# rapidsai/distributed-join

Hardware: NVIDIA H100
Metric: joined rows/sec (build+probe rows through distributed_inner_join) at 400Mx400M int64 (higher is better)
Workload: dtype int64

## Files before the change

### distributed-join_b200/csrc/join.cu

```cuda
#include <algorithm>
#include <cstdlib>
#include <type_traits>

#include "dj_device.cuh"
#include "dj_internal.h"

namespace dj {

namespace {

template <int THREADS, int SLOTS, int BUILD_CHUNK, int TARGET_ROWS, int PROBE_STAGES, int OUT_ROWS>
struct JoinCfg {
  static constexpr int kThreads     = THREADS;
  static constexpr int kConsumers   = THREADS - 32;
  static constexpr int kConsWarps   = kConsumers / 32;
  static constexpr int kSlots       = SLOTS;
  static constexpr int kBuildChunk  = BUILD_CHUNK;
  static constexpr int kTargetRows  = TARGET_ROWS;
  static constexpr int kProbeChunk  = kConsumers;
  static constexpr int kProbeStages = PROBE_STAGES;
  static constexpr int kOutRows     = OUT_ROWS;
};
using CfgA = JoinCfg<1024, 8192, 1792, 1536, 2, 576>;
using CfgB = JoinCfg<512, 4096, 1024, 768, 2, 256>;

constexpr int kOutTiles    = 3;
constexpr int kDescBuckets = 128;

struct JoinDev {
  const Row* build;
  const int64_t *bbeg, *bend;
  const Row* probe;
  const int64_t *pbeg, *pend;
  int nbuckets;
  int64_t* out[4];
  int64_t out_capacity;
  unsigned long long* out_count;
  uint32_t* probe_bits;
  uint8_t* out_sides;
  uint32_t* build_bits;
};

constexpr int kInner = 0, kSemi = DJ_JOIN_LEFT_SEMI, kAnti = DJ_JOIN_LEFT_ANTI;
constexpr int kLeftOuter = DJ_JOIN_LEFT_OUTER, kFullOuter = DJ_JOIN_FULL_OUTER, kMark = kJoinFullOuterMark;
constexpr uint8_t kSideProbe = DJ_SIDE_LEFT, kSideBuild = DJ_SIDE_RIGHT;

__host__ __device__ constexpr bool is_outer(int kind)
{
  return kind == kLeftOuter || kind == kFullOuter || kind == kMark;
}
__host__ __device__ constexpr bool marks_build(int kind) { return kind == kFullOuter || kind == kMark; }

template <class C>
struct __align__(128) JoinSmem {
  uint32_t slots[2][C::kSlots];
  Row brow[2][C::kBuildChunk];
  Row prow[C::kProbeStages][C::kProbeChunk];
  int64_t sout[kOutTiles][4][C::kOutRows];
  int64_t dbb[kDescBuckets], dbe[kDescBuckets];
  int64_t dpb[kDescBuckets], dpe[kDescBuckets];
  unsigned long long full_build[2], empty_build[2];
  unsigned long long full_probe[C::kProbeStages], empty_probe[C::kProbeStages];
  unsigned long long sbase[kOutTiles];
  int scnt[kOutTiles];
};

template <class C>
struct __align__(128) OuterJoinSmem : JoinSmem<C> {
  uint8_t ssides[kOutTiles][C::kOutRows];
  uint32_t bmatch[2][C::kBuildChunk / 32];
};

template <class C, int KIND>
using JoinSmemOf = std::conditional_t<is_outer(KIND), OuterJoinSmem<C>, JoinSmem<C>>;

template <int N>
__device__ __forceinline__ void consumer_sync()
{
  asm volatile("bar.sync 1, %0;" ::"n"(N) : "memory");
}

template <int KIND, class S>
__device__ __forceinline__ int next_valid_bucket(const S& s, int lb, int nd)
{
  if constexpr (KIND == kAnti || KIND == kLeftOuter || KIND == kMark) {
    while (lb < nd && s.dpe[lb] == s.dpb[lb]) lb++;
  } else if constexpr (KIND == kFullOuter) {
    while (lb < nd && s.dbe[lb] == s.dbb[lb] && s.dpe[lb] == s.dpb[lb]) lb++;
  } else {
    while (lb < nd && (s.dbe[lb] == s.dbb[lb] || s.dpe[lb] == s.dpb[lb])) lb++;
  }
  return lb;
}

__device__ __forceinline__ uint32_t slot_tag(uint32_t h) { return 0x100000u | (h >> 12); }

template <class C>
__device__ __forceinline__ void emit_outer_row(OuterJoinSmem<C>& s, const JoinDev& d, int cur, int lane, bool emit,
                                               int64_t bk, int64_t bp, int64_t pk, int64_t pv, uint8_t sides)
{
  const unsigned m = __ballot_sync(0xffffffffu, emit);
  if (m == 0) return;
  const int leader = __ffs(m) - 1;
  int obase        = 0;
  if (lane == leader) {
    obase = atomicAdd(&s.scnt[cur], __popc(m));
    if (obase >= C::kOutRows) atomicSub(&s.scnt[cur], __popc(m));
  }
  obase            = __shfl_sync(0xffffffffu, obase, leader);
  const int pos    = obase + __popc(m & lanemask_lt());
  const bool spill = emit && pos >= C::kOutRows;
  if (emit && !spill) {
    s.sout[cur][0][pos] = bk;
    s.sout[cur][1][pos] = bp;
    s.sout[cur][2][pos] = pk;
    s.sout[cur][3][pos] = pv;
    s.ssides[cur][pos]  = sides;
  }
  const unsigned ms = __ballot_sync(0xffffffffu, spill);
  if (ms) {
    const int sl         = __ffs(ms) - 1;
    unsigned long long g = 0;
    if (lane == sl) g = atomicAdd(d.out_count, (unsigned long long)__popc(ms));
    g = __shfl_sync(0xffffffffu, g, sl);
    if (spill) {
      const int64_t gi = (int64_t)g + __popc(ms & lanemask_lt());
      if (gi < d.out_capacity) {
        d.out[0][gi]     = bk;
        d.out[1][gi]     = bp;
        d.out[2][gi]     = pk;
        d.out[3][gi]     = pv;
        d.out_sides[gi]  = sides;
      }
    }
  }
}

template <class C, int KIND>
__global__ void __launch_bounds__(C::kThreads, 1) bucket_join_kernel(JoinDev d)
{
  using Smem = JoinSmemOf<C, KIND>;
  constexpr int kConsumers = C::kConsumers;
  constexpr bool kOuter    = is_outer(KIND);
  constexpr bool kEmptyJob = KIND == kAnti || kOuter;
  constexpr int kCols      = (KIND == kSemi || KIND == kAnti) ? 2 : 4;
  extern __shared__ __align__(128) unsigned char smem_raw[];
  Smem& s        = *reinterpret_cast<Smem*>(smem_raw);
  const int tid  = threadIdx.x;
  const int lane = tid & 31;
  const int warp = tid >> 5;
  const bool is_producer = warp == C::kConsWarps;

  if (tid == 0) {
    for (int i = 0; i < 2; i++) {
      mbar_init(&s.full_build[i], 1);
      mbar_init(&s.empty_build[i], C::kConsWarps);
    }
    for (int i = 0; i < C::kProbeStages; i++) {
      mbar_init(&s.full_probe[i], 1);
      mbar_init(&s.empty_probe[i], C::kConsWarps);
    }
    for (int i = 0; i < kOutTiles; i++) s.scnt[i] = 0;
    asm volatile("fence.mbarrier_init.release.cluster;" ::: "memory");
  }
  for (int i = tid; i < 2 * C::kSlots; i += C::kThreads) (&s.slots[0][0])[i] = 0;
  if constexpr (marks_build(KIND))
    for (int i = tid; i < 2 * (C::kBuildChunk / 32); i += C::kThreads) (&s.bmatch[0][0])[i] = 0;
  __syncthreads();

  const int lo = (int)((int64_t)d.nbuckets * blockIdx.x / gridDim.x);
  const int hi = (int)((int64_t)d.nbuckets * (blockIdx.x + 1) / gridDim.x);

  uint32_t q = 0;
  uint32_t u = 0;
  int cur = 0, pend_tile = 0, pend_n = 0;
  unsigned long long pend_base_reg = 0;

  for (int base = lo; base < hi; base += kDescBuckets) {
    const int nd = min(kDescBuckets, hi - base);
    __syncthreads();
    for (int i = tid; i < nd; i += C::kThreads) {
      s.dbb[i] = d.bbeg[base + i];
      s.dbe[i] = d.bend[base + i];
      s.dpb[i] = d.pbeg[base + i];
      s.dpe[i] = d.pend[base + i];
    }
    __syncthreads();

    if (is_producer) {
      if (lane == 0) {
        for (int lb = next_valid_bucket<KIND>(s, 0, nd); lb < nd; lb = next_valid_bucket<KIND>(s, lb + 1, nd)) {
          const int64_t b0 = s.dbb[lb], b1 = s.dbe[lb], p0 = s.dpb[lb], p1 = s.dpe[lb];
          for (int64_t c0 = b0; c0 < b1 || (kEmptyJob && c0 == b0); c0 += C::kBuildChunk) {
            {
              const int bs = u & 1;
              const int n  = (int)min((int64_t)C::kBuildChunk, b1 - c0);
              mbar_wait(&s.empty_build[bs], ((u >> 1) & 1) ^ 1);
              mbar_expect_tx(&s.full_build[bs], (uint32_t)n * 16u);
              if (!kEmptyJob || n > 0) tma_load(s.brow[bs], d.build + c0, (uint32_t)n * 16u, &s.full_build[bs]);
              u++;
            }
            for (int64_t r0 = p0; r0 < p1; r0 += C::kProbeChunk) {
              const int st = q % C::kProbeStages;
              const int n  = (int)min((int64_t)C::kProbeChunk, p1 - r0);
              mbar_wait(&s.empty_probe[st], ((q / C::kProbeStages) & 1) ^ 1);
              mbar_expect_tx(&s.full_probe[st], (uint32_t)n * 16u);
              tma_load(s.prow[st], d.probe + r0, (uint32_t)n * 16u, &s.full_probe[st]);
              q++;
            }
          }
        }
      }
      __syncwarp();
    } else {
      for (int lb = next_valid_bucket<KIND>(s, 0, nd); lb < nd; lb = next_valid_bucket<KIND>(s, lb + 1, nd)) {
        const int64_t b0 = s.dbb[lb], b1 = s.dbe[lb], p0 = s.dpb[lb], p1 = s.dpe[lb];
        const bool multi = KIND != kInner && b1 - b0 > C::kBuildChunk;
        for (int64_t c0 = b0; c0 < b1 || (kEmptyJob && c0 == b0); c0 += C::kBuildChunk) {
          const bool last = c0 + C::kBuildChunk >= b1;
          const int bs = u & 1;
          const int nb = (int)min((int64_t)C::kBuildChunk, b1 - c0);
          uint32_t* slots     = s.slots[bs];
          const Row* brow     = s.brow[bs];
          mbar_wait(&s.full_build[bs], (u >> 1) & 1);
          for (int r = tid; r < nb; r += kConsumers) {
            const uint32_t h = slot_hash_i64(brow[r].key);
            const uint32_t e = (slot_tag(h) << 11) | (uint32_t)r;
            uint32_t slot    = h & (C::kSlots - 1);
            while (atomicCAS(&slots[slot], 0u, e) != 0u) slot = (slot + 1) & (C::kSlots - 1);
          }
          {
            uint4* other = reinterpret_cast<uint4*>(s.slots[bs ^ 1]);
            for (int i = tid; i < C::kSlots / 4; i += kConsumers) other[i] = make_uint4(0, 0, 0, 0);
            if constexpr (KIND == kFullOuter)
              for (int i = tid; i < C::kBuildChunk / 32; i += kConsumers) s.bmatch[bs ^ 1][i] = 0;
          }
          consumer_sync<kConsumers>();

          for (int64_t r0 = p0; r0 < p1; r0 += C::kProbeChunk) {
            const int st = q % C::kProbeStages;
            const int np = (int)min((int64_t)C::kProbeChunk, p1 - r0);
            mbar_wait(&s.full_probe[st], (q / C::kProbeStages) & 1);
            bool alive = tid < np;
            int64_t k = 0, v = 0;
            if (alive) {
              const int4 pr = *reinterpret_cast<const int4*>(&s.prow[st][tid]);
              k = (int64_t)(((uint64_t)(uint32_t)pr.y << 32) | (uint32_t)pr.x);
              v = (int64_t)(((uint64_t)(uint32_t)pr.w << 32) | (uint32_t)pr.z);
            }
            const unsigned landed =
              __reduce_and_sync(0xffffffffu, (uint32_t)((uint64_t)k ^ ((uint64_t)k >> 32) ^ (uint64_t)v ^
                                                        ((uint64_t)v >> 32)) | 1u);
            if (lane == 0 && landed) mbar_arrive(&s.empty_probe[st]);
            q++;

            const uint32_t h    = slot_hash_i64(k);
            const uint32_t want = slot_tag(h);
            uint32_t slot       = h & (C::kSlots - 1);
            if constexpr (kOuter) {
              const bool valid = alive;
              bool matched     = false;
              while (true) {
                bool found = false;
                int idx    = 0;
                if (alive) {
                  while (true) {
                    const uint32_t e = slots[slot];
                    if (e == 0u) {
                      alive = false;
                      break;
                    }
                    if ((e >> 11) == want) {
                      idx = (int)(e & 0x7ffu);
                      if (brow[idx].key == k) {
                        found = true;
                        break;
                      }
                    }
                    slot = (slot + 1) & (C::kSlots - 1);
                  }
                }
                if (!__any_sync(0xffffffffu, found)) break;
                int64_t bpay = 0;
                if (found) {
                  matched = true;
                  bpay    = brow[idx].pay;
                  if constexpr (marks_build(KIND)) {
                    uint32_t* w      = &s.bmatch[bs][idx >> 5];
                    const uint32_t b = 1u << (idx & 31);
                    if (!(*w & b)) atomicOr(w, b);
                  }
                }
                emit_outer_row<C>(s, d, cur, lane, found, k, bpay, k, v, kSideBuild | kSideProbe);
                if (found) slot = (slot + 1) & (C::kSlots - 1);
              }
              const int64_t prow_at = r0 + tid;
              uint32_t* word        = d.probe_bits + (prow_at >> 5);
              const uint32_t bit    = 1u << (prow_at & 31);
              if (multi && matched && !last) atomicOr(word, bit);
              const bool lone = valid && !matched && last && (!multi || !(__ldcg(word) & bit));
              emit_outer_row<C>(s, d, cur, lane, lone, 0, 0, k, v, kSideProbe);
              continue;
            }
            if constexpr (KIND == kSemi || KIND == kAnti) {
              bool found = false;
              if (alive) {
                while (true) {
                  const uint32_t e = slots[slot];
                  if (e == 0u) break;
                  if ((e >> 11) == want && brow[e & 0x7ffu].key == k) {
                    found = true;
                    break;
                  }
                  slot = (slot + 1) & (C::kSlots - 1);
                }
              }
              const int64_t prow_at = r0 + tid;
              uint32_t* word        = d.probe_bits + (prow_at >> 5);
              const uint32_t bit    = 1u << (prow_at & 31);
              bool emit;
              if constexpr (KIND == kSemi) {
                emit = found && (!multi || !(atomicOr(word, bit) & bit));
              } else {
                if (multi && found && !last) atomicOr(word, bit);
                emit = alive && !found && last && (!multi || !(__ldcg(word) & bit));
              }
              const unsigned m = __ballot_sync(0xffffffffu, emit);
              if (m) {
                const int leader = __ffs(m) - 1;
                int obase        = 0;
                if (lane == leader) {
                  obase = atomicAdd(&s.scnt[cur], __popc(m));
                  if (obase >= C::kOutRows) atomicSub(&s.scnt[cur], __popc(m));
                }
                obase            = __shfl_sync(0xffffffffu, obase, leader);
                const int pos    = obase + __popc(m & lanemask_lt());
                const bool spill = emit && pos >= C::kOutRows;
                if (emit && !spill) {
                  s.sout[cur][0][pos] = k;
                  s.sout[cur][1][pos] = v;
                }
                const unsigned ms = __ballot_sync(0xffffffffu, spill);
                if (ms) {
                  const int sl = __ffs(ms) - 1;
                  unsigned long long g = 0;
                  if (lane == sl) g = atomicAdd(d.out_count, (unsigned long long)__popc(ms));
                  g = __shfl_sync(0xffffffffu, g, sl);
                  if (spill) {
                    const int64_t gi = (int64_t)g + __popc(ms & lanemask_lt());
                    if (gi < d.out_capacity) {
                      d.out[0][gi] = k;
                      d.out[1][gi] = v;
                    }
                  }
                }
              }
              continue;
            }
            while (true) {
              bool found = false;
              int idx    = 0;
              if (alive) {
                while (true) {
                  const uint32_t e = slots[slot];
                  if (e == 0u) {
                    alive = false;
                    break;
                  }
                  if ((e >> 11) == want) {
                    idx = (int)(e & 0x7ffu);
                    if (brow[idx].key == k) {
                      found = true;
                      break;
                    }
                  }
                  slot = (slot + 1) & (C::kSlots - 1);
                }
              }
              const unsigned m = __ballot_sync(0xffffffffu, found);
              if (m == 0) break;
              const int leader = __ffs(m) - 1;
              int obase        = 0;
              if (lane == leader) {
                obase = atomicAdd(&s.scnt[cur], __popc(m));
                if (obase >= C::kOutRows) atomicSub(&s.scnt[cur], __popc(m));
              }
              obase         = __shfl_sync(0xffffffffu, obase, leader);
              const int pos = obase + __popc(m & lanemask_lt());
              const bool spill = found && pos >= C::kOutRows;
              if (found && !spill) {
                s.sout[cur][0][pos] = k;
                s.sout[cur][1][pos] = brow[idx].pay;
                s.sout[cur][2][pos] = k;
                s.sout[cur][3][pos] = v;
              }
              const unsigned ms = __ballot_sync(0xffffffffu, spill);
              if (ms) {
                const int sl = __ffs(ms) - 1;
                unsigned long long g = 0;
                if (lane == sl) g = atomicAdd(d.out_count, (unsigned long long)__popc(ms));
                g = __shfl_sync(0xffffffffu, g, sl);
                if (spill) {
                  const int64_t gi = (int64_t)g + __popc(ms & lanemask_lt());
                  if (gi < d.out_capacity) {
                    d.out[0][gi] = k;
                    d.out[1][gi] = brow[idx].pay;
                    d.out[2][gi] = k;
                    d.out[3][gi] = v;
                  }
                }
              }
              if (found) slot = (slot + 1) & (C::kSlots - 1);
            }
          }

          if (tid == 0 && pend_n) s.sbase[pend_tile] = pend_base_reg;
          consumer_sync<kConsumers>();
          if constexpr (KIND == kFullOuter) {
            for (int r0 = tid - lane; r0 < nb; r0 += kConsumers) {
              const int r     = r0 + lane;
              const bool lone = r < nb && !((s.bmatch[bs][r >> 5] >> (r & 31)) & 1u);
              int64_t bk = 0, bp = 0;
              if (lone) {
                bk = brow[r].key;
                bp = brow[r].pay;
              }
              emit_outer_row<C>(s, d, cur, lane, lone, bk, bp, 0, 0, kSideBuild);
            }
            consumer_sync<kConsumers>();
          }
          if constexpr (KIND == kMark) {
            if (tid < C::kBuildChunk / 32) {
              const uint32_t w = s.bmatch[bs][tid];
              if (w) {
                s.bmatch[bs][tid] = 0;
                const int64_t at  = c0 + 32 * tid;
                uint32_t* g       = d.build_bits + (at >> 5);
                const int sh      = (int)(at & 31);
                atomicOr(g, w << sh);
                if (sh && (w >> (32 - sh))) atomicOr(g + 1, w >> (32 - sh));
              }
            }
          }
          if (lane == 0) mbar_arrive(&s.empty_build[bs]);
          if (pend_n) {
            const int64_t gb = (int64_t)s.sbase[pend_tile];
#pragma unroll
            for (int c = 0; c < kCols; c++)
              for (int i = tid; i < pend_n; i += kConsumers)
                if (gb + i < d.out_capacity) d.out[c][gb + i] = s.sout[pend_tile][c][i];
            if constexpr (kOuter)
              for (int i = tid; i < pend_n; i += kConsumers)
                if (gb + i < d.out_capacity) d.out_sides[gb + i] = s.ssides[pend_tile][i];
            if (tid == 0) s.scnt[pend_tile] = 0;
            pend_n = 0;
          }
          int n_out = s.scnt[cur];
          if (n_out > 0) {
            if (n_out > C::kOutRows) n_out = C::kOutRows;
            if (tid == 0) pend_base_reg = atomicAdd(d.out_count, (unsigned long long)n_out);
            pend_n    = n_out;
            pend_tile = cur;
            cur       = cur + 1 == kOutTiles ? 0 : cur + 1;
          }
          u++;
        }
      }
    }
  }

  if (!is_producer) {
    if (tid == 0 && pend_n) s.sbase[pend_tile] = pend_base_reg;
    consumer_sync<kConsumers>();
    if (pend_n) {
      const int64_t gb = (int64_t)s.sbase[pend_tile];
#pragma unroll
      for (int c = 0; c < kCols; c++)
        for (int i = tid; i < pend_n; i += kConsumers)
          if (gb + i < d.out_capacity) d.out[c][gb + i] = s.sout[pend_tile][c][i];
      if constexpr (kOuter)
        for (int i = tid; i < pend_n; i += kConsumers)
          if (gb + i < d.out_capacity) d.out_sides[gb + i] = s.ssides[pend_tile][i];
    }
  }
}

int join_shape()
{
  static int shape = -1;
  if (shape < 0) {
    const char* e = getenv("DJ_JOIN_SHAPE");
    shape         = (e && (e[0] == 'B' || e[0] == 'b')) ? 1 : 0;
  }
  return shape;
}

template <class C, int KIND>
int launch_join(const JoinDev& d, int ctas_per_sm, cudaStream_t stream)
{
  const size_t smem = sizeof(JoinSmemOf<C, KIND>);
  auto kern         = bucket_join_kernel<C, KIND>;
  DJ_CUDA_TRY(cudaFuncSetAttribute(kern, cudaFuncAttributeMaxDynamicSharedMemorySize, (int)smem));
  int grid = sm_count() * ctas_per_sm;
  if (grid > d.nbuckets) grid = d.nbuckets;
  {
    ProfScope prof(DJ_PROF_JOIN, stream);
    kern<<<grid, C::kThreads, smem, stream>>>(d);
  }
  DJ_LAUNCH_CHECK();
  return DJ_OK;
}

template <class C>
int launch_join_kind(const JoinDev& d, int kind, int ctas_per_sm, cudaStream_t stream)
{
  return kind == kSemi        ? launch_join<C, kSemi>(d, ctas_per_sm, stream)
         : kind == kAnti      ? launch_join<C, kAnti>(d, ctas_per_sm, stream)
         : kind == kLeftOuter ? launch_join<C, kLeftOuter>(d, ctas_per_sm, stream)
         : kind == kFullOuter ? launch_join<C, kFullOuter>(d, ctas_per_sm, stream)
         : kind == kMark      ? launch_join<C, kMark>(d, ctas_per_sm, stream)
                              : launch_join<C, kInner>(d, ctas_per_sm, stream);
}

constexpr int kAppendChunk = 4096;

__global__ void __launch_bounds__(256) append_rows_kernel(const Row* rows, const int64_t* sb, const int64_t* se,
                                                          int64_t* out_key, int64_t* out_pay, int64_t* null_key,
                                                          int64_t* null_pay, uint8_t* out_sides, uint8_t sides,
                                                          int64_t out_capacity, unsigned long long* out_count)
{
  __shared__ unsigned long long base;
  const int64_t b = sb[blockIdx.y], e = se[blockIdx.y];
  for (int64_t c0 = b + (int64_t)blockIdx.x * kAppendChunk; c0 < e; c0 += (int64_t)gridDim.x * kAppendChunk) {
    const int n = (int)min((int64_t)kAppendChunk, e - c0);
    __syncthreads();
    if (threadIdx.x == 0) base = atomicAdd(out_count, (unsigned long long)n);
    __syncthreads();
    for (int i = threadIdx.x; i < n; i += blockDim.x) {
      const int64_t g = (int64_t)base + i;
      if (g < out_capacity) {
        const Row r = rows[c0 + i];
        out_key[g]  = r.key;
        out_pay[g]  = r.pay;
        if (out_sides) {
          null_key[g]  = 0;
          null_pay[g]  = 0;
          out_sides[g] = sides;
        }
      }
    }
  }
}

constexpr int kEmitThreads = 256, kEmitPerThread = 4, kEmitTile = kEmitThreads * kEmitPerThread;

__global__ void __launch_bounds__(kEmitThreads) emit_unmatched_build_kernel(
  const Row* rows, const int64_t* bbeg, const int64_t* bend, int nbuckets, const uint32_t* bits, int64_t* null_key,
  int64_t* null_pay, int64_t* out_key, int64_t* out_pay, uint8_t* out_sides, int64_t out_capacity,
  unsigned long long* out_count)
{
  constexpr int kRuns = kEmitTile / 32;
  __shared__ unsigned long long run_base[kRuns];
  __shared__ int run_cnt[kRuns];
  const int lane = threadIdx.x & 31, warp = threadIdx.x >> 5;
  for (int b = blockIdx.x; b < nbuckets; b += gridDim.x) {
    const int64_t b0 = bbeg[b], b1 = bend[b];
    for (int64_t t0 = b0; t0 < b1; t0 += kEmitTile) {
      int4 row[kEmitPerThread];
      unsigned lone[kEmitPerThread];
#pragma unroll
      for (int j = 0; j < kEmitPerThread; j++) {
        const int64_t r = t0 + j * kEmitThreads + threadIdx.x;
        bool mine       = false;
        row[j]          = make_int4(0, 0, 0, 0);
        if (r < b1 && !((bits[r >> 5] >> (r & 31)) & 1u)) {
          mine   = true;
          row[j] = __ldg(reinterpret_cast<const int4*>(rows + r));
        }
        lone[j] = __ballot_sync(0xffffffffu, mine);
        if (lane == 0) run_cnt[j * (kEmitThreads / 32) + warp] = __popc(lone[j]);
      }
      __syncthreads();
      if (warp == 0) {
        int c[kRuns / 32], sum = 0;
#pragma unroll
        for (int i = 0; i < kRuns / 32; i++) {
          c[i] = run_cnt[lane * (kRuns / 32) + i];
          sum += c[i];
        }
        int incl = sum;
#pragma unroll
        for (int o = 1; o < 32; o <<= 1) {
          const int v = __shfl_up_sync(0xffffffffu, incl, o);
          if (lane >= o) incl += v;
        }
        const int total      = __shfl_sync(0xffffffffu, incl, 31);
        unsigned long long g = 0;
        if (lane == 0 && total) g = atomicAdd(out_count, (unsigned long long)total);
        g = __shfl_sync(0xffffffffu, g, 0) + (unsigned long long)(incl - sum);
#pragma unroll
        for (int i = 0; i < kRuns / 32; i++) {
          run_base[lane * (kRuns / 32) + i] = g;
          g += c[i];
        }
      }
      __syncthreads();
#pragma unroll
      for (int j = 0; j < kEmitPerThread; j++) {
        if (!((lone[j] >> lane) & 1u)) continue;
        const int64_t g = (int64_t)run_base[j * (kEmitThreads / 32) + warp] + __popc(lone[j] & lanemask_lt());
        if (g < out_capacity) {
          null_key[g]  = 0;
          null_pay[g]  = 0;
          out_key[g]   = (int64_t)(((uint64_t)(uint32_t)row[j].y << 32) | (uint32_t)row[j].x);
          out_pay[g]   = (int64_t)(((uint64_t)(uint32_t)row[j].w << 32) | (uint32_t)row[j].z);
          out_sides[g] = kSideBuild;
        }
      }
    }
  }
}

}

RadixPlan make_radix_plan(int64_t nbuild)
{
  const int target = join_shape() == 1 ? CfgB::kTargetRows : CfgA::kTargetRows;
  RadixPlan p{0, 0, 1};
  int bits = 0;
  while (bits < 20 && (nbuild >> bits) > target) bits++;
  if (bits <= 10) {
    p.bits1 = bits;
    p.bits2 = 0;
  } else {
    p.bits1 = bits / 2;
    p.bits2 = bits - p.bits1;
  }
  p.nbuckets = 1 << bits;
  return p;
}

int run_bucket_join(const JoinBuffers& jb, bool swap_output_sides, cudaStream_t stream)
{
  JoinDev d{};
  d.build    = jb.build;
  d.bbeg     = jb.d_build_begin;
  d.bend     = jb.d_build_end;
  d.probe    = jb.probe;
  d.pbeg     = jb.d_probe_begin;
  d.pend     = jb.d_probe_end;
  d.nbuckets = jb.nbuckets;
  for (int c = 0; c < 4; c++) d.out[c] = jb.out[swap_output_sides ? (c + 2) % 4 : c];
  d.out_capacity = jb.out_capacity;
  d.out_count    = (unsigned long long*)jb.d_out_count;
  d.probe_bits   = jb.d_probe_bits;
  d.out_sides    = jb.out_sides;
  d.build_bits   = jb.d_build_bits;
  return join_shape() == 1 ? launch_join_kind<CfgB>(d, jb.kind, 2, stream)
                           : launch_join_kind<CfgA>(d, jb.kind, 1, stream);
}

int append_segment_rows(const Row* rows, const int64_t* d_seg_begin, const int64_t* d_seg_end, int nseg,
                        int64_t max_seg_rows, int64_t* out_key, int64_t* out_pay, int64_t out_capacity,
                        int64_t* d_out_count, cudaStream_t stream, int64_t* null_key, int64_t* null_pay,
                        uint8_t* out_sides, uint8_t sides)
{
  if (nseg <= 0 || max_seg_rows <= 0) return DJ_OK;
  const int64_t chunks = (max_seg_rows + kAppendChunk - 1) / kAppendChunk;
  const dim3 grid((unsigned)(chunks < 64 ? chunks : 64), (unsigned)nseg);
  {
    ProfScope prof(DJ_PROF_OTHER, stream);
    append_rows_kernel<<<grid, 256, 0, stream>>>(rows, d_seg_begin, d_seg_end, out_key, out_pay, null_key, null_pay,
                                                 out_sides, sides, out_capacity, (unsigned long long*)d_out_count);
  }
  DJ_LAUNCH_CHECK();
  return DJ_OK;
}

int emit_unmatched_build(const Row* rows, const int64_t* d_begin, const int64_t* d_end, int nbuckets,
                         const uint32_t* d_build_bits, int64_t* const out[4], uint8_t* out_sides,
                         int64_t out_capacity, int64_t* d_out_count, cudaStream_t stream)
{
  if (nbuckets <= 0) return DJ_OK;
  const int grid = std::min(nbuckets, sm_count() * 8);
  {
    ProfScope prof(DJ_PROF_OTHER, stream);
    emit_unmatched_build_kernel<<<grid, kEmitThreads, 0, stream>>>(rows, d_begin, d_end, nbuckets, d_build_bits, out[0],
                                                                   out[1], out[2], out[3], out_sides, out_capacity,
                                                                   (unsigned long long*)d_out_count);
  }
  DJ_LAUNCH_CHECK();
  return DJ_OK;
}

const void* join_module_kernel() { return (const void*)bucket_join_kernel<CfgA, kInner>; }

}
```

Measured before the change: 25.06 billion.

## Split join CTA into independent producer/consumer groups processing interleaved buckets

Reorganizes the bucket join kernel so that a 1024-thread CTA becomes two independent 512-thread groups. Each group has its own hash slots, build buffer, probe stages, mbarriers and output tile, and takes every other valid bucket. Double-buffered build chunks and the three-tile output ring are replaced by one buffer per group, with the output tile flushed at the start of the next chunk. The aim is to cut CTA-wide synchronisation and let two pipelines overlap their latency, at the cost of losing build double-buffering within a group and adding more serialising group barriers.

```diff
diff --git a/distributed-join_b200/csrc/join.cu b/distributed-join_b200/csrc/join.cu
--- a/distributed-join_b200/csrc/join.cu
+++ b/distributed-join_b200/csrc/join.cu
@@ -9,22 +9,23 @@
 
 namespace {
 
-template <int THREADS, int SLOTS, int BUILD_CHUNK, int TARGET_ROWS, int PROBE_STAGES, int OUT_ROWS>
+template <int GROUPS, int SLOTS, int BUILD_CHUNK, int TARGET_ROWS, int PROBE_STAGES, int OUT_ROWS>
 struct JoinCfg {
-  static constexpr int kThreads     = THREADS;
-  static constexpr int kConsumers   = THREADS - 32;
-  static constexpr int kConsWarps   = kConsumers / 32;
-  static constexpr int kSlots       = SLOTS;
-  static constexpr int kBuildChunk  = BUILD_CHUNK;
-  static constexpr int kTargetRows  = TARGET_ROWS;
-  static constexpr int kProbeChunk  = kConsumers;
-  static constexpr int kProbeStages = PROBE_STAGES;
-  static constexpr int kOutRows     = OUT_ROWS;
+  static constexpr int kGroups       = GROUPS;
+  static constexpr int kGroupThreads = 512;
+  static constexpr int kThreads      = GROUPS * kGroupThreads;
+  static constexpr int kConsumers    = kGroupThreads - 32;
+  static constexpr int kConsWarps    = kConsumers / 32;
+  static constexpr int kSlots        = SLOTS;
+  static constexpr int kBuildChunk   = BUILD_CHUNK;
+  static constexpr int kTargetRows   = TARGET_ROWS;
+  static constexpr int kProbeChunk   = kConsumers;
+  static constexpr int kProbeStages  = PROBE_STAGES;
+  static constexpr int kOutRows      = OUT_ROWS;
 };
-using CfgA = JoinCfg<1024, 8192, 1792, 1536, 2, 576>;
-using CfgB = JoinCfg<512, 4096, 1024, 768, 2, 256>;
-
-constexpr int kOutTiles    = 3;
+using CfgA = JoinCfg<2, 8192, 1792, 1536, 2, 1024>;
+using CfgB = JoinCfg<1, 4096, 1024, 768, 2, 512>;
+
 constexpr int kDescBuckets = 128;
 
 struct JoinDev {
@@ -52,32 +53,40 @@
 __host__ __device__ constexpr bool marks_build(int kind) { return kind == kFullOuter || kind == kMark; }
 
 template <class C>
+struct __align__(128) JoinGroup {
+  uint32_t slots[C::kSlots];
+  Row brow[C::kBuildChunk];
+  Row prow[C::kProbeStages][C::kProbeChunk];
+  int64_t sout[4][C::kOutRows];
+  unsigned long long full_build, empty_build;
+  unsigned long long full_probe[C::kProbeStages], empty_probe[C::kProbeStages];
+  unsigned long long sbase;
+  int scnt;
+};
+
+template <class C>
+struct __align__(128) OuterJoinGroup : JoinGroup<C> {
+  uint8_t ssides[C::kOutRows];
+  uint32_t bmatch[C::kBuildChunk / 32];
+};
+
+template <class C, int KIND>
+using JoinGroupOf = std::conditional_t<is_outer(KIND), OuterJoinGroup<C>, JoinGroup<C>>;
+
+template <class C, int KIND>
 struct __align__(128) JoinSmem {
-  uint32_t slots[2][C::kSlots];
-  Row brow[2][C::kBuildChunk];
-  Row prow[C::kProbeStages][C::kProbeChunk];
-  int64_t sout[kOutTiles][4][C::kOutRows];
+  JoinGroupOf<C, KIND> grp[C::kGroups];
   int64_t dbb[kDescBuckets], dbe[kDescBuckets];
   int64_t dpb[kDescBuckets], dpe[kDescBuckets];
-  unsigned long long full_build[2], empty_build[2];
-  unsigned long long full_probe[C::kProbeStages], empty_probe[C::kProbeStages];
-  unsigned long long sbase[kOutTiles];
-  int scnt[kOutTiles];
 };
 
-template <class C>
-struct __align__(128) OuterJoinSmem : JoinSmem<C> {
-  uint8_t ssides[kOutTiles][C::kOutRows];
-  uint32_t bmatch[2][C::kBuildChunk / 32];
-};
-
-template <class C, int KIND>
-using JoinSmemOf = std::conditional_t<is_outer(KIND), OuterJoinSmem<C>, JoinSmem<C>>;
-
 template <int N>
-__device__ __forceinline__ void consumer_sync()
-{
-  asm volatile("bar.sync 1, %0;" ::"n"(N) : "memory");
+__device__ __forceinline__ void group_sync(int g)
+{
+  if (g == 0)
+    asm volatile("bar.sync 1, %0;" ::"n"(N) : "memory");
+  else
+    asm volatile("bar.sync 2, %0;" ::"n"(N) : "memory");
 }
 
 template <int KIND, class S>
@@ -93,10 +102,18 @@
   return lb;
 }
 
+template <class C, int KIND, class S>
+__device__ __forceinline__ int next_group_bucket(const S& s, int lb, int nd, uint32_t& ord, int g)
+{
+  for (lb = next_valid_bucket<KIND>(s, lb, nd); lb < nd; lb = next_valid_bucket<KIND>(s, lb + 1, nd))
+    if (ord++ % C::kGroups == (uint32_t)g) break;
+  return lb;
+}
+
 __device__ __forceinline__ uint32_t slot_tag(uint32_t h) { return 0x100000u | (h >> 12); }
 
 template <class C>
-__device__ __forceinline__ void emit_outer_row(OuterJoinSmem<C>& s, const JoinDev& d, int cur, int lane, bool emit,
+__device__ __forceinline__ void emit_outer_row(OuterJoinGroup<C>& s, const JoinDev& d, int lane, bool emit,
                                                int64_t bk, int64_t bp, int64_t pk, int64_t pv, uint8_t sides)
 {
   const unsigned m = __ballot_sync(0xffffffffu, emit);
@@ -104,18 +121,18 @@
   const int leader = __ffs(m) - 1;
   int obase        = 0;
   if (lane == leader) {
-    obase = atomicAdd(&s.scnt[cur], __popc(m));
-    if (obase >= C::kOutRows) atomicSub(&s.scnt[cur], __popc(m));
+    obase = atomicAdd(&s.scnt, __popc(m));
+    if (obase >= C::kOutRows) atomicSub(&s.scnt, __popc(m));
   }
   obase            = __shfl_sync(0xffffffffu, obase, leader);
   const int pos    = obase + __popc(m & lanemask_lt());
   const bool spill = emit && pos >= C::kOutRows;
   if (emit && !spill) {
-    s.sout[cur][0][pos] = bk;
-    s.sout[cur][1][pos] = bp;
-    s.sout[cur][2][pos] = pk;
-    s.sout[cur][3][pos] = pv;
-    s.ssides[cur][pos]  = sides;
+    s.sout[0][pos] = bk;
+    s.sout[1][pos] = bp;
+    s.sout[2][pos] = pk;
+    s.sout[3][pos] = pv;
+    s.ssides[pos]  = sides;
   }
   const unsigned ms = __ballot_sync(0xffffffffu, spill);
   if (ms) {
@@ -137,44 +154,57 @@
 }
 
 template <class C, int KIND>
+__device__ __forceinline__ void copy_out_tile(const JoinGroupOf<C, KIND>& s, const JoinDev& d, int n, int ltid)
+{
+  constexpr int kCols = (KIND == kSemi || KIND == kAnti) ? 2 : 4;
+  const int64_t gb    = (int64_t)s.sbase;
+#pragma unroll
+  for (int c = 0; c < kCols; c++)
+    for (int i = ltid; i < n; i += C::kConsumers)
+      if (gb + i < d.out_capacity) d.out[c][gb + i] = s.sout[c][i];
+  if constexpr (is_outer(KIND))
+    for (int i = ltid; i < n; i += C::kConsumers)
+      if (gb + i < d.out_capacity) d.out_sides[gb + i] = s.ssides[i];
+}
+
+template <class C, int KIND>
 __global__ void __launch_bounds__(C::kThreads, 1) bucket_join_kernel(JoinDev d)
 {
-  using Smem = JoinSmemOf<C, KIND>;
+  using Smem = JoinSmem<C, KIND>;
   constexpr int kConsumers = C::kConsumers;
   constexpr bool kOuter    = is_outer(KIND);
   constexpr bool kEmptyJob = KIND == kAnti || kOuter;
-  constexpr int kCols      = (KIND == kSemi || KIND == kAnti) ? 2 : 4;
   extern __shared__ __align__(128) unsigned char smem_raw[];
   Smem& s        = *reinterpret_cast<Smem*>(smem_raw);
   const int tid  = threadIdx.x;
   const int lane = tid & 31;
-  const int warp = tid >> 5;
-  const bool is_producer = warp == C::kConsWarps;
-
-  if (tid == 0) {
-    for (int i = 0; i < 2; i++) {
-      mbar_init(&s.full_build[i], 1);
-      mbar_init(&s.empty_build[i], C::kConsWarps);
+  const int g    = tid / C::kGroupThreads;
+  const int ltid = tid % C::kGroupThreads;
+  const bool is_producer = ltid >= kConsumers;
+  auto& sg = s.grp[g];
+
+  if (ltid == 0) {
+    mbar_init(&sg.full_build, 1);
+    mbar_init(&sg.empty_build, C::kConsWarps);
+    for (int i = 0; i < C::kProbeStages; i++) {
+      mbar_init(&sg.full_probe[i], 1);
+      mbar_init(&sg.empty_probe[i], C::kConsWarps);
     }
-    for (int i = 0; i < C::kProbeStages; i++) {
-      mbar_init(&s.full_probe[i], 1);
-      mbar_init(&s.empty_probe[i], C::kConsWarps);
-    }
-    for (int i = 0; i < kOutTiles; i++) s.scnt[i] = 0;
+    sg.scnt = 0;
     asm volatile("fence.mbarrier_init.release.cluster;" ::: "memory");
   }
-  for (int i = tid; i < 2 * C::kSlots; i += C::kThreads) (&s.slots[0][0])[i] = 0;
+  for (int i = ltid; i < C::kSlots; i += C::kGroupThreads) sg.slots[i] = 0;
   if constexpr (marks_build(KIND))
-    for (int i = tid; i < 2 * (C::kBuildChunk / 32); i += C::kThreads) (&s.bmatch[0][0])[i] = 0;
+    for (int i = ltid; i < C::kBuildChunk / 32; i += C::kGroupThreads) sg.bmatch[i] = 0;
   __syncthreads();
 
   const int lo = (int)((int64_t)d.nbuckets * blockIdx.x / gridDim.x);
   const int hi = (int)((int64_t)d.nbuckets * (blockIdx.x + 1) / gridDim.x);
 
-  uint32_t q = 0;
-  uint32_t u = 0;
-  int cur = 0, pend_tile = 0, pend_n = 0;
-  unsigned long long pend_base_reg = 0;
+  uint32_t ord = 0;
+  uint32_t q   = 0;
+  uint32_t u   = 0;
+  int pend_n = 0;
 
   for (int base = lo; base < hi; base += kDescBuckets) {
     const int nd = min(kDescBuckets, hi - base);
@@ -189,23 +219,23 @@
 
     if (is_producer) {
       if (lane == 0) {
-        for (int lb = next_valid_bucket<KIND>(s, 0, nd); lb < nd; lb = next_valid_bucket<KIND>(s, lb + 1, nd)) {
+        for (int lb = next_group_bucket<C, KIND>(s, 0, nd, ord, g); lb < nd;
+             lb     = next_group_bucket<C, KIND>(s, lb + 1, nd, ord, g)) {
           const int64_t b0 = s.dbb[lb], b1 = s.dbe[lb], p0 = s.dpb[lb], p1 = s.dpe[lb];
           for (int64_t c0 = b0; c0 < b1 || (kEmptyJob && c0 == b0); c0 += C::kBuildChunk) {
             {
-              const int bs = u & 1;
-              const int n  = (int)min((int64_t)C::kBuildChunk, b1 - c0);
-              mbar_wait(&s.empty_build[bs], ((u >> 1) & 1) ^ 1);
-              mbar_expect_tx(&s.full_build[bs], (uint32_t)n * 16u);
-              if (!kEmptyJob || n > 0) tma_load(s.brow[bs], d.build + c0, (uint32_t)n * 16u, &s.full_build[bs]);
+              const int n = (int)min((int64_t)C::kBuildChunk, b1 - c0);
+              mbar_wait(&sg.empty_build, (u & 1) ^ 1);
+              mbar_expect_tx(&sg.full_build, (uint32_t)n * 16u);
+              if (!kEmptyJob || n > 0) tma_load(sg.brow, d.build + c0, (uint32_t)n * 16u, &sg.full_build);
               u++;
             }
             for (int64_t r0 = p0; r0 < p1; r0 += C::kProbeChunk) {
               const int st = q % C::kProbeStages;
               const int n  = (int)min((int64_t)C::kProbeChunk, p1 - r0);
-              mbar_wait(&s.empty_probe[st], ((q / C::kProbeStages) & 1) ^ 1);
-              mbar_expect_tx(&s.full_probe[st], (uint32_t)n * 16u);
-              tma_load(s.prow[st], d.probe + r0, (uint32_t)n * 16u, &s.full_probe[st]);
+              mbar_wait(&sg.empty_probe[st], ((q / C::kProbeStages) & 1) ^ 1);
+              mbar_expect_tx(&sg.full_probe[st], (uint32_t)n * 16u);
+              tma_load(sg.prow[st], d.probe + r0, (uint32_t)n * 16u, &sg.full_probe[st]);
               q++;
             }
           }
@@ -213,45 +243,45 @@
       }
       __syncwarp();
     } else {
-      for (int lb = next_valid_bucket<KIND>(s, 0, nd); lb < nd; lb = next_valid_bucket<KIND>(s, lb + 1, nd)) {
+      uint32_t* const slots = sg.slots;
+      const Row* const brow = sg.brow;
+      for (int lb = next_group_bucket<C, KIND>(s, 0, nd, ord, g); lb < nd;
+           lb     = next_group_bucket<C, KIND>(s, lb + 1, nd, ord, g)) {
         const int64_t b0 = s.dbb[lb], b1 = s.dbe[lb], p0 = s.dpb[lb], p1 = s.dpe[lb];
         const bool multi = KIND != kInner && b1 - b0 > C::kBuildChunk;
         for (int64_t c0 = b0; c0 < b1 || (kEmptyJob && c0 == b0); c0 += C::kBuildChunk) {
           const bool last = c0 + C::kBuildChunk >= b1;
-          const int bs = u & 1;
           const int nb = (int)min((int64_t)C::kBuildChunk, b1 - c0);
-          uint32_t* slots     = s.slots[bs];
-          const Row* brow     = s.brow[bs];
-          mbar_wait(&s.full_build[bs], (u >> 1) & 1);
-          for (int r = tid; r < nb; r += kConsumers) {
+          group_sync<kConsumers>(g);
+          if (pend_n) {
+            copy_out_tile<C, KIND>(sg, d, pend_n, ltid);
+            if (ltid == 0) sg.scnt = 0;
+            pend_n = 0;
+          }
+          mbar_wait(&sg.full_build, u & 1);
+          for (int r = ltid; r < nb; r += kConsumers) {
             const uint32_t h = slot_hash_i64(brow[r].key);
             const uint32_t e = (slot_tag(h) << 11) | (uint32_t)r;
             uint32_t slot    = h & (C::kSlots - 1);
             while (atomicCAS(&slots[slot], 0u, e) != 0u) slot = (slot + 1) & (C::kSlots - 1);
           }
-          {
-            uint4* other = reinterpret_cast<uint4*>(s.slots[bs ^ 1]);
-            for (int i = tid; i < C::kSlots / 4; i += kConsumers) other[i] = make_uint4(0, 0, 0, 0);
-            if constexpr (KIND == kFullOuter)
-              for (int i = tid; i < C::kBuildChunk / 32; i += kConsumers) s.bmatch[bs ^ 1][i] = 0;
-          }
-          consumer_sync<kConsumers>();
+          group_sync<kConsumers>(g);
 
           for (int64_t r0 = p0; r0 < p1; r0 += C::kProbeChunk) {
             const int st = q % C::kProbeStages;
             const int np = (int)min((int64_t)C::kProbeChunk, p1 - r0);
-            mbar_wait(&s.full_probe[st], (q / C::kProbeStages) & 1);
-            bool alive = tid < np;
+            mbar_wait(&sg.full_probe[st], (q / C::kProbeStages) & 1);
+            bool alive = ltid < np;
             int64_t k = 0, v = 0;
             if (alive) {
-              const int4 pr = *reinterpret_cast<const int4*>(&s.prow[st][tid]);
+              const int4 pr = *reinterpret_cast<const int4*>(&sg.prow[st][ltid]);
               k = (int64_t)(((uint64_t)(uint32_t)pr.y << 32) | (uint32_t)pr.x);
               v = (int64_t)(((uint64_t)(uint32_t)pr.w << 32) | (uint32_t)pr.z);
             }
             const unsigned landed =
               __reduce_and_sync(0xffffffffu, (uint32_t)((uint64_t)k ^ ((uint64_t)k >> 32) ^ (uint64_t)v ^
                                                         ((uint64_t)v >> 32)) | 1u);
-            if (lane == 0 && landed) mbar_arrive(&s.empty_probe[st]);
+            if (lane == 0 && landed) mbar_arrive(&sg.empty_probe[st]);
             q++;
 
             const uint32_t h    = slot_hash_i64(k);
@@ -286,20 +316,20 @@
                   matched = true;
                   bpay    = brow[idx].pay;
                   if constexpr (marks_build(KIND)) {
-                    uint32_t* w      = &s.bmatch[bs][idx >> 5];
+                    uint32_t* w      = &sg.bmatch[idx >> 5];
                     const uint32_t b = 1u << (idx & 31);
                     if (!(*w & b)) atomicOr(w, b);
                   }
                 }
-                emit_outer_row<C>(s, d, cur, lane, found, k, bpay, k, v, kSideBuild | kSideProbe);
+                emit_outer_row<C>(sg, d, lane, found, k, bpay, k, v, kSideBuild | kSideProbe);
                 if (found) slot = (slot + 1) & (C::kSlots - 1);
               }
-              const int64_t prow_at = r0 + tid;
+              const int64_t prow_at = r0 + ltid;
               uint32_t* word        = d.probe_bits + (prow_at >> 5);
               const uint32_t bit    = 1u << (prow_at & 31);
               if (multi && matched && !last) atomicOr(word, bit);
               const bool lone = valid && !matched && last && (!multi || !(__ldcg(word) & bit));
-              emit_outer_row<C>(s, d, cur, lane, lone, 0, 0, k, v, kSideProbe);
+              emit_outer_row<C>(sg, d, lane, lone, 0, 0, k, v, kSideProbe);
               continue;
             }
             if constexpr (KIND == kSemi || KIND == kAnti) {
@@ -315,7 +345,7 @@
                   slot = (slot + 1) & (C::kSlots - 1);
                 }
               }
-              const int64_t prow_at = r0 + tid;
+              const int64_t prow_at = r0 + ltid;
               uint32_t* word        = d.probe_bits + (prow_at >> 5);
               const uint32_t bit    = 1u << (prow_at & 31);
               bool emit;
@@ -330,24 +360,24 @@
                 const int leader = __ffs(m) - 1;
                 int obase        = 0;
                 if (lane == leader) {
-                  obase = atomicAdd(&s.scnt[cur], __popc(m));
-                  if (obase >= C::kOutRows) atomicSub(&s.scnt[cur], __popc(m));
+                  obase = atomicAdd(&sg.scnt, __popc(m));
+                  if (obase >= C::kOutRows) atomicSub(&sg.scnt, __popc(m));
                 }
                 obase            = __shfl_sync(0xffffffffu, obase, leader);
                 const int pos    = obase + __popc(m & lanemask_lt());
                 const bool spill = emit && pos >= C::kOutRows;
                 if (emit && !spill) {
-                  s.sout[cur][0][pos] = k;
-                  s.sout[cur][1][pos] = v;
+                  sg.sout[0][pos] = k;
+                  sg.sout[1][pos] = v;
                 }
                 const unsigned ms = __ballot_sync(0xffffffffu, spill);
                 if (ms) {
                   const int sl = __ffs(ms) - 1;
-                  unsigned long long g = 0;
-                  if (lane == sl) g = atomicAdd(d.out_count, (unsigned long long)__popc(ms));
-                  g = __shfl_sync(0xffffffffu, g, sl);
+                  unsigned long long gc = 0;
+                  if (lane == sl) gc = atomicAdd(d.out_count, (unsigned long long)__popc(ms));
+                  gc = __shfl_sync(0xffffffffu, gc, sl);
                   if (spill) {
-                    const int64_t gi = (int64_t)g + __popc(ms & lanemask_lt());
+                    const int64_t gi = (int64_t)gc + __popc(ms & lanemask_lt());
                     if (gi < d.out_capacity) {
                       d.out[0][gi] = k;
                       d.out[1][gi] = v;
@@ -382,26 +412,26 @@
               const int leader = __ffs(m) - 1;
               int obase        = 0;
               if (lane == leader) {
-                obase = atomicAdd(&s.scnt[cur], __popc(m));
-                if (obase >= C::kOutRows) atomicSub(&s.scnt[cur], __popc(m));
+                obase = atomicAdd(&sg.scnt, __popc(m));
+                if (obase >= C::kOutRows) atomicSub(&sg.scnt, __popc(m));
               }
               obase         = __shfl_sync(0xffffffffu, obase, leader);
               const int pos = obase + __popc(m & lanemask_lt());
               const bool spill = found && pos >= C::kOutRows;
               if (found && !spill) {
-                s.sout[cur][0][pos] = k;
-                s.sout[cur][1][pos] = brow[idx].pay;
-                s.sout[cur][2][pos] = k;
-                s.sout[cur][3][pos] = v;
+                sg.sout[0][pos] = k;
+                sg.sout[1][pos] = brow[idx].pay;
+                sg.sout[2][pos] = k;
+                sg.sout[3][pos] = v;
               }
               const unsigned ms = __ballot_sync(0xffffffffu, spill);
               if (ms) {
                 const int sl = __ffs(ms) - 1;
-                unsigned long long g = 0;
-                if (lane == sl) g = atomicAdd(d.out_count, (unsigned long long)__popc(ms));
-                g = __shfl_sync(0xffffffffu, g, sl);
+                unsigned long long gc = 0;
+                if (lane == sl) gc = atomicAdd(d.out_count, (unsigned long long)__popc(ms));
+                gc = __shfl_sync(0xffffffffu, gc, sl);
                 if (spill) {
-                  const int64_t gi = (int64_t)g + __popc(ms & lanemask_lt());
+                  const int64_t gi = (int64_t)gc + __popc(ms & lanemask_lt());
                   if (gi < d.out_capacity) {
                     d.out[0][gi] = k;
                     d.out[1][gi] = brow[idx].pay;
@@ -414,55 +444,45 @@
             }
           }
 
-          if (tid == 0 && pend_n) s.sbase[pend_tile] = pend_base_reg;
-          consumer_sync<kConsumers>();
+          group_sync<kConsumers>(g);
           if constexpr (KIND == kFullOuter) {
-            for (int r0 = tid - lane; r0 < nb; r0 += kConsumers) {
+            for (int r0 = ltid - lane; r0 < nb; r0 += kConsumers) {
               const int r     = r0 + lane;
-              const bool lone = r < nb && !((s.bmatch[bs][r >> 5] >> (r & 31)) & 1u);
+              const bool lone = r < nb && !((sg.bmatch[r >> 5] >> (r & 31)) & 1u);
               int64_t bk = 0, bp = 0;
               if (lone) {
                 bk = brow[r].key;
                 bp = brow[r].pay;
               }
-              emit_outer_row<C>(s, d, cur, lane, lone, bk, bp, 0, 0, kSideBuild);
+              emit_outer_row<C>(sg, d, lane, lone, bk, bp, 0, 0, kSideBuild);
             }
-            consumer_sync<kConsumers>();
+            group_sync<kConsumers>(g);
+            for (int i = ltid; i < C::kBuildChunk / 32; i += kConsumers) sg.bmatch[i] = 0;
           }
           if constexpr (KIND == kMark) {
-            if (tid < C::kBuildChunk / 32) {
-              const uint32_t w = s.bmatch[bs][tid];
+            if (ltid < C::kBuildChunk / 32) {
+              const uint32_t w = sg.bmatch[ltid];
               if (w) {
-                s.bmatch[bs][tid] = 0;
-                const int64_t at  = c0 + 32 * tid;
-                uint32_t* g       = d.build_bits + (at >> 5);
-                const int sh      = (int)(at & 31);
-                atomicOr(g, w << sh);
-                if (sh && (w >> (32 - sh))) atomicOr(g + 1, w >> (32 - sh));
+                sg.bmatch[ltid]  = 0;
+                const int64_t at = c0 + 32 * ltid;
+                uint32_t* gw     = d.build_bits + (at >> 5);
+                const int sh     = (int)(at & 31);
+                atomicOr(gw, w << sh);
+                if (sh && (w >> (32 - sh))) atomicOr(gw + 1, w >> (32 - sh));
               }
             }
           }
-          if (lane == 0) mbar_arrive(&s.empty_build[bs]);
-          if (pend_n) {
-            const int64_t gb = (int64_t)s.sbase[pend_tile];
-#pragma unroll
-            for (int c = 0; c < kCols; c++)
-              for (int i = tid; i < pend_n; i += kConsumers)
-                if (gb + i < d.out_capacity) d.out[c][gb + i] = s.sout[pend_tile][c][i];
-            if constexpr (kOuter)
-              for (int i = tid; i < pend_n; i += kConsumers)
-                if (gb + i < d.out_capacity) d.out_sides[gb + i] = s.ssides[pend_tile][i];
-            if (tid == 0) s.scnt[pend_tile] = 0;
-            pend_n = 0;
+          if (lane == 0) mbar_arrive(&sg.empty_build);
+          int n_out = sg.scnt;
+          if (n_out > C::kOutRows) n_out = C::kOutRows;
+          unsigned long long tile_base = 0;
+          if (ltid == 0 && n_out > 0) tile_base = atomicAdd(d.out_count, (unsigned long long)n_out);
+          {
+            uint4* t = reinterpret_cast<uint4*>(slots);
+            for (int i = ltid; i < C::kSlots / 4; i += kConsumers) t[i] = make_uint4(0, 0, 0, 0);
           }
-          int n_out = s.scnt[cur];
-          if (n_out > 0) {
-            if (n_out > C::kOutRows) n_out = C::kOutRows;
-            if (tid == 0) pend_base_reg = atomicAdd(d.out_count, (unsigned long long)n_out);
-            pend_n    = n_out;
-            pend_tile = cur;
-            cur       = cur + 1 == kOutTiles ? 0 : cur + 1;
-          }
+          if (ltid == 0 && n_out > 0) sg.sbase = tile_base;
+          pend_n = n_out;
           u++;
         }
       }
@@ -470,18 +490,8 @@
   }
 
   if (!is_producer) {
-    if (tid == 0 && pend_n) s.sbase[pend_tile] = pend_base_reg;
-    consumer_sync<kConsumers>();
-    if (pend_n) {
-      const int64_t gb = (int64_t)s.sbase[pend_tile];
-#pragma unroll
-      for (int c = 0; c < kCols; c++)
-        for (int i = tid; i < pend_n; i += kConsumers)
-          if (gb + i < d.out_capacity) d.out[c][gb + i] = s.sout[pend_tile][c][i];
-      if constexpr (kOuter)
-        for (int i = tid; i < pend_n; i += kConsumers)
-          if (gb + i < d.out_capacity) d.out_sides[gb + i] = s.ssides[pend_tile][i];
-    }
+    group_sync<kConsumers>(g);
+    if (pend_n) copy_out_tile<C, KIND>(sg, d, pend_n, ltid);
   }
 }
 
@@ -498,7 +508,8 @@
 template <class C, int KIND>
 int launch_join(const JoinDev& d, int ctas_per_sm, cudaStream_t stream)
 {
-  const size_t smem = sizeof(JoinSmemOf<C, KIND>);
+  const size_t smem = sizeof(JoinSmem<C, KIND>);
+  static_assert(sizeof(JoinSmem<C, KIND>) <= 227 * 1024, "more shared memory than a block may use");
   auto kern         = bucket_join_kernel<C, KIND>;
   DJ_CUDA_TRY(cudaFuncSetAttribute(kern, cudaFuncAttributeMaxDynamicSharedMemorySize, (int)smem));
   int grid = sm_count() * ctas_per_sm;
```

Measured after the change: 26.49 billion, median of 6. +5.7%, better.
